# rchikhi/rust-seq2kminmers

Hardware: AMD Instinct MI355X
Metric: input bases/s (Gbp/s) for k-min-mer extraction, l=31 k=10 d=0.01 (higher is better)
Workload: dtype u32

## Files before the change

rust-seq2kminmers_amd/csrc/s2k_tile_impl.h:

```cpp
#pragma once
#include "s2k_dev.h"
#include "s2k_static_l.h"

#include <cstdlib>
#include <mutex>
#include <type_traits>

namespace s2k {
namespace {

#ifndef S2K_TW
#define S2K_TW 12
#endif
#ifndef S2K_TW_REG
#ifdef S2K_PROFILE
#define S2K_TW_REG 12
#else
#define S2K_TW_REG 16
#endif
#endif
template <bool HPC> constexpr int tw() { return HPC ? S2K_TW : S2K_TW_REG; }
template <bool HPC> constexpr int waves_per_simd() { return tw<HPC>() / 4; }
static_assert(S2K_TW % 4 == 0 && S2K_TW_REG % 4 == 0, "whole waves per SIMD");
constexpr int HS_OFF = 16;
constexpr int BUF_BYTES = HS_OFF + TILE_BASES + 128;
#ifndef S2K_CAPP
#define S2K_CAPP 16
#endif
constexpr int CAPP = S2K_CAPP;
constexpr int NPC = TILE_T / CAPP;
constexpr int MAX_L_TILED = 64;
#ifndef S2K_LISTCAP
#define S2K_LISTCAP 256
#endif
#ifndef S2K_JOBCAP
#define S2K_JOBCAP 32
#endif
#ifndef S2K_REDERIVE_GROUP
#define S2K_REDERIVE_GROUP 8
#endif
constexpr int LISTCAP_REG = S2K_TW_REG > 12 ? 216 : S2K_LISTCAP;
constexpr int LISTCAP_HPC = 192;
template <bool HPC> constexpr int listcap() { return HPC ? LISTCAP_HPC : LISTCAP_REG; }
template <bool HPC> constexpr int jobcap() { return !HPC && S2K_TW_REG > 12 ? 16 : S2K_JOBCAP; }
#ifndef S2K_REG_LA
#define S2K_REG_LA 1
#endif
#ifndef S2K_HPC_LA
#define S2K_HPC_LA 2
#endif
constexpr int REG_LA = S2K_REG_LA;
constexpr int HPC_LA = S2K_HPC_LA;
constexpr int NBL = 32;
template <bool DESC> constexpr int stores_per_round() { return DESC ? 1 : 3; }
static_assert(NBL == META_SEGS, "TileMeta keeps NBL segment starts");
constexpr int NPRE = 10;

#ifndef S2K_SD_SHIFT
#define S2K_SD_SHIFT 6
#endif
constexpr int ROW_W = 6, ROW_PFX = 4, ROW_CUM = 5, N_ROWS = 66, SD_SHIFT = S2K_SD_SHIFT;
struct HpcLds {
    uint32_t row[N_ROWS][ROW_W];
    uint32_t halo_pos[64];
    uint8_t sd[SD_SHIFT == 6 ? 160 : 288];
};
static_assert(sizeof(HpcLds) % 16 == 0, "the tile buffer behind it is read 16 bytes at a time");
struct NoHpcLds {};

template <bool HPC>
struct alignas(16) WaveLdsT : std::conditional<HPC, HpcLds, NoHpcLds>::type {
    uint8_t buf[BUF_BYTES];
    uint16_t list[listcap<HPC>()];
    uint16_t jobx[jobcap<HPC>()];
    uint16_t jobslot[jobcap<HPC>()];
    int16_t hb[NBL];
    uint16_t rs16[NBL];
};
#ifdef S2K_PROFILE
typedef __attribute__((address_space(3))) unsigned long long *ph_ptr_t;
constexpr int PROFILE_LDS_BYTES = 16 * 16 * 8;
#else
typedef uint64_t *ph_ptr_t;
constexpr int PROFILE_LDS_BYTES = 0;
#endif
constexpr int SEED_TABLE_BYTES = 2 * 256 * 8;
#ifndef S2K_SEL8
#define S2K_SEL8 1
#endif
constexpr int TABLE_BYTES = SEED_TABLE_BYTES;
constexpr int SEL8_OFF = SEED_TABLE_BYTES, SEL8_BYTES = S2K_SEL8 ? 256 * 8 : 0;
#ifndef S2K_PASS2_ACC
#define S2K_PASS2_ACC 1
#endif
static_assert(!S2K_PASS2_ACC || S2K_SEL8, "pass 2 reads its v_perm_b32 selectors from sel8");
#ifndef S2K_LPH
#define S2K_LPH 0
#endif
#ifndef S2K_WARM2
#define S2K_WARM2 1
#endif
constexpr int WARM_OFF = SEL8_OFF + SEL8_BYTES, WARM_BYTES = S2K_WARM2 ? 256 * 8 : 0;
template <bool HPC> constexpr int table_bytes() { return SEED_TABLE_BYTES + (HPC ? SEL8_BYTES + WARM_BYTES : 0); }
template <bool HPC>
constexpr int block_lds_bytes() { return table_bytes<HPC>() + tw<HPC>() * (int)sizeof(WaveLdsT<HPC>) + PROFILE_LDS_BYTES; }
#ifndef S2K_EXPERIMENT
static_assert(block_lds_bytes<true>() <= 160 * 1024 && block_lds_bytes<false>() <= 160 * 1024, "the block of a CU must fit its 160 KiB of LDS");
#endif

__device__ inline uint32_t wave_incl_scan(uint32_t v, int lane) {
    (void)lane;
    uint32_t t;
    t = (uint32_t)__builtin_amdgcn_update_dpp(0, (int)v, 0x111, 0xf, 0xf, false);
    uint32_t a = v + t;
    t = (uint32_t)__builtin_amdgcn_update_dpp(0, (int)v, 0x112, 0xf, 0xf, false);
    a += t;
    t = (uint32_t)__builtin_amdgcn_update_dpp(0, (int)v, 0x113, 0xf, 0xf, false);
    a += t;
// ... 6 lines not shown
    t = (uint32_t)__builtin_amdgcn_update_dpp(0, (int)a, 0x143, 0xc, 0xf, false);
    a += t;
    return a;
}
__device__ inline uint32_t wave_incl_max(uint32_t v) {
    uint32_t t, a;
    t = (uint32_t)__builtin_amdgcn_update_dpp(0, (int)v, 0x111, 0xf, 0xf, false);
    a = v > t ? v : t;
    t = (uint32_t)__builtin_amdgcn_update_dpp(0, (int)v, 0x112, 0xf, 0xf, false);
    a = a > t ? a : t;
    t = (uint32_t)__builtin_amdgcn_update_dpp(0, (int)v, 0x113, 0xf, 0xf, false);
    a = a > t ? a : t;
    t = (uint32_t)__builtin_amdgcn_update_dpp(0, (int)a, 0x114, 0xf, 0xe, false);
    a = a > t ? a : t;
    t = (uint32_t)__builtin_amdgcn_update_dpp(0, (int)a, 0x118, 0xf, 0xc, false);
    a = a > t ? a : t;
    t = (uint32_t)__builtin_amdgcn_update_dpp(0, (int)a, 0x142, 0xa, 0xf, false);
    a = a > t ? a : t;
    t = (uint32_t)__builtin_amdgcn_update_dpp(0, (int)a, 0x143, 0xc, 0xf, false);
    a = a > t ? a : t;
    return a;
}
__device__ inline uint32_t bcast(uint32_t v, int src) {
    return (uint32_t)__builtin_amdgcn_readlane((int)v, __builtin_amdgcn_readfirstlane(src));
}

__device__ inline uint32_t select_nth_32(uint32_t w, uint32_t n) {
    uint32_t r = 0, c;
    c = __popc(w & 0xFFFFu); if (n >= c) { n -= c; r += 16; w >>= 16; }
    c = __popc(w & 0xFFu);   if (n >= c) { n -= c; r += 8;  w >>= 8; }
    c = __popc(w & 0xFu);    if (n >= c) { n -= c; r += 4;  w >>= 4; }
    c = __popc(w & 0x3u);    if (n >= c) { n -= c; r += 2;  w >>= 2; }
    c = w & 1u;              if (n >= c) { r += 1; }
    return r;
}
__device__ __forceinline__ uint32_t select_nth_32_lut(uint32_t w, uint32_t n) {
    typedef __attribute__((address_space(3))) const uint8_t *lds_cu8;
    uint32_t r = 0, c;
    c = __popc(w & 0xFFFFu); if (n >= c) { n -= c; r += 16; w >>= 16; }
    c = __popc(w & 0xFFu);   if (n >= c) { n -= c; r += 8;  w >>= 8; }
    return r + reinterpret_cast<lds_cu8>((uint32_t)SEL8_OFF)[8u * (w & 0xFFu) + n];
}
__device__ __forceinline__ uint32_t mad24(uint32_t a, uint32_t b, uint32_t c) {
    uint32_t r;
    asm("v_mad_u32_u24 %0, %1, %2, %3" : "=v"(r) : "v"(a), "s"(b), "v"(c));
    return r;
}
__device__ __forceinline__ uint32_t div_tq(uint32_t x, uint32_t rcp) { return __umul24(x >> 4, rcp) >> 16; }
static_assert(TILE_T == 144, "div_tile_t's reciprocal is that of 144");
__device__ __forceinline__ uint32_t div_tile_t(uint32_t x) { return __umul24(x, 3641u) >> 19; }
__device__ __forceinline__ uint32_t bits_below(int v) {
    const int t = v < 0 ? 0 : (v > 32 ? 32 : v);
    return (uint32_t)(1ull << (uint32_t)t) - 1u;
}
__device__ __forceinline__ uint32_t heads_before_word(uint32_t cum, uint32_t g) {
    return __builtin_amdgcn_perm(cum, 0u, g + 0x0C0C0C03u);
}
__device__ __forceinline__ uint32_t word_of_head(uint32_t cum, uint32_t n) {
    uint32_t g = 0;
    asm("v_cmp_ge_u32_sdwa vcc, %1, %2 src0_sel:DWORD src1_sel:BYTE_0\n\t"
        "v_addc_co_u32_e32 %0, vcc, 0, %0, vcc\n\t"
        "v_cmp_ge_u32_sdwa vcc, %1, %2 src0_sel:DWORD src1_sel:BYTE_1\n\t"
        "v_addc_co_u32_e32 %0, vcc, 0, %0, vcc\n\t"
        "v_cmp_ge_u32_sdwa vcc, %1, %2 src0_sel:DWORD src1_sel:BYTE_2\n\t"
        "v_addc_co_u32_e32 %0, vcc, 0, %0, vcc\n\t"
        "v_cmp_ge_u32_sdwa vcc, %1, %2 src0_sel:DWORD src1_sel:BYTE_3\n\t"
        "v_addc_co_u32_e32 %0, vcc, 0, %0, vcc"
        : "+v"(g)
        : "v"(n), "v"(cum)
        : "vcc");
    return g;
}
template <int BYTE>
__device__ __forceinline__ uint32_t byte_x8(uint32_t w) {
    uint32_t off;
    if constexpr (BYTE == 0) asm("v_lshlrev_b32_sdwa %0, %1, %2 dst_sel:DWORD dst_unused:UNUSED_PAD src0_sel:DWORD src1_sel:BYTE_0" : "=v"(off) : "v"(3u), "v"(w));
    if constexpr (BYTE == 1) asm("v_lshlrev_b32_sdwa %0, %1, %2 dst_sel:DWORD dst_unused:UNUSED_PAD src0_sel:DWORD src1_sel:BYTE_1" : "=v"(off) : "v"(3u), "v"(w));
    if constexpr (BYTE == 2) asm("v_lshlrev_b32_sdwa %0, %1, %2 dst_sel:DWORD dst_unused:UNUSED_PAD src0_sel:DWORD src1_sel:BYTE_2" : "=v"(off) : "v"(3u), "v"(w));
    if constexpr (BYTE == 3) asm("v_lshlrev_b32_sdwa %0, %1, %2 dst_sel:DWORD dst_unused:UNUSED_PAD src0_sel:DWORD src1_sel:BYTE_3" : "=v"(off) : "v"(3u), "v"(w));
    return off;
}
template <int TABLE_OFF>
__device__ __forceinline__ uint2 seed_pair(uint32_t off) {
#ifdef HX_NOLDS
    return make_uint2(off, off);
#endif
    typedef __attribute__((address_space(3))) const unsigned long long lds_cu64;
    const unsigned long long v = *reinterpret_cast<lds_cu64 *>(off + TABLE_OFF);
    return make_uint2((uint32_t)v, (uint32_t)(v >> 32));
}
__device__ __forceinline__ uint2 tab_in(const uint2 *tab, uint32_t c) { return tab[c]; }
__device__ __forceinline__ uint2 tab_out(const uint2 *tab, uint32_t c) { return tab[256 + c]; }

__device__ __forceinline__ void hit_track(uint32_t hv, uint32_t bound, uint32_t &cap, uint32_t &bits) {
#ifdef HX_NOTRACK
    bits ^= hv;
    return;
#endif
    asm("v_cmp_ge_u32_e32 vcc, %2, %3\n\t"
        "v_cndmask_b32_e32 %0, %0, %3, vcc\n\t"
        "v_addc_co_u32_e32 %1, vcc, %1, %1, vcc"
        : "+v"(cap), "+v"(bits)
        : "s"(bound), "v"(hv)
        : "vcc");
}
template <int P>
// ... 513 lines not shown
__device__ __forceinline__ uint32_t heads_before_raw(const WL &S, uint32_t rel) {
    const uint32_t o = div_tile_t(rel), wi = rel - __umul24(o, (uint32_t)TILE_T), g = wi >> 5;
    const uint2 pc = *reinterpret_cast<const uint2 *>(&S.row[o][ROW_PFX]);
    const uint32_t wd = S.row[o][g];
    return (pc.x >> 16) + heads_before_word(pc.y, g) + __popc(wd & ((1u << (wi & 31u)) - 1u));
}

__device__ __forceinline__ uint32_t lookback_heads(const uint32_t *W, uint64_t t, int lane, Counts *counts, uint32_t early, bool &dead) {
    uint32_t sum = 0;
    if (dead) return 0;
    for (uint64_t tb = t;;) {
        const bool exists = tb >= 1 + (uint64_t)lane;
        const uint32_t *p = W + (exists ? tb - 1 - (uint64_t)lane : 0);
        uint32_t w = HW_VALID;
        int fs = 64;
        for (int polls = 0;; polls++) {
            if (exists) w = (polls == 0 && tb == t) ? early : __hip_atomic_load(p, __ATOMIC_RELAXED, __HIP_MEMORY_SCOPE_AGENT);
            const uint64_t valid = __ballot((w & HW_VALID) != 0u);
            const uint64_t stop = __ballot((w & HW_VALID) != 0u && (w & HW_PASS) == 0u);
            fs = stop ? __builtin_ctzll(stop) : 64;
            const uint64_t need = fs >= 63 ? ~0ull : ((2ull << fs) - 1ull);
            if ((valid & need) == need) break;
            const bool anybody = (polls & 63) == 63 && __hip_atomic_load(&counts->need_runs, __ATOMIC_RELAXED, __HIP_MEMORY_SCOPE_AGENT) != 0u;
            if (polls >= 4096 || __builtin_amdgcn_readfirstlane((int)anybody)) {
                if (lane == 0) counts->need_runs = 1;
                dead = true;
                return 0;
            }
            __builtin_amdgcn_s_sleep(16);
        }
        const uint32_t mine = (lane <= fs) ? (w & HW_COUNT) : 0u;
        sum += bcast(wave_incl_scan(mine, lane), 63);
        if (fs < 64) break;
        tb -= 64;
    }
    return sum;
}

template <class WL>
__device__ __forceinline__ void publish_tile_heads(uint32_t *W, uint64_t t, const WL &S, uint32_t nh, uint64_t t0, uint32_t tile_len,
                                                   bool any_start, uint64_t last_start, bool first_begins_here, int lane) {
    uint32_t word;
    if (!any_start) {
        word = HW_VALID | (first_begins_here ? 0u : HW_PASS) | nh;
    } else if (last_start >= t0 + tile_len) {
        word = HW_VALID;
    } else {
        const uint32_t c = heads_before_raw(S, (uint32_t)(last_start - t0));
        word = HW_VALID | (nh - c);
    }
    if (lane == 0) __hip_atomic_store(W + t, word, __ATOMIC_RELAXED, __HIP_MEMORY_SCOPE_AGENT);
}

template <int L, bool HPC, bool DESC, class WL, class IssueNext>
__device__ __forceinline__ uint32_t dense_phase(IssueNext &&issue_next, WL &S, const uint8_t *D, const uint2 *tab,
                                                const uint64_t *__restrict__ read_off, uint64_t n_reads, uint64_t t,
                                                uint64_t t0, uint32_t tile_len, uint32_t nh, uint32_t halo_n,
                                                uint32_t Tq, uint32_t rcpTq, uint32_t l, uint32_t r0, uint32_t r1, uint64_t bpos0,
                                                uint64_t rs0, int lane, const Records &rec, uint64_t *pool_cursor,
                                                uint32_t *mn_cnt, Counts *counts, uint64_t &base, const Sem &sem,
                                                unsigned long long *__restrict__ d_agg, TileMeta *__restrict__ d_meta, uint32_t K1,
                                                const uint32_t (&caps)[NPC], const uint32_t (&raw)[5], uint32_t lb_early,
                                                bool &lb_dead, ph_ptr_t ph, uint64_t &stamp) {
    constexpr int LISTCAP = listcap<HPC>();
    const uint32_t wclr = HPC ? (sem.keep_last ? l - 1 : l) : l - 1;
    const uint32_t tql = __umul24(Tq, (uint32_t)lane);
    uint32_t vm[5];
    {
        int vc = (int)nh - (int)tql;
#pragma unroll
        for (int d = 0; d < 5; d++) {
            vm[d] = raw[d] & bits_below(vc - 32 * d);
        }
    }
    const uint64_t tile_end = t0 + tile_len;
    uint32_t nb = 0;
    const bool many = (r1 - r0) > (uint32_t)(NBL - 2);
    bool ext_at_end = false;
    {
        uint64_t bpos = bpos0;
        uint64_t chunk_prev = rs0;
        int32_t hb_carry = 0;
        for (uint32_t c0 = 0;; c0 += 64) {
            const bool internal = bpos > t0 && bpos < tile_end;
            const bool external = bpos >= tile_end;
            const uint64_t em = __ballot(external);
            const int first_ext = em ? __builtin_ctzll(em) : 64;
            int32_t HB = 0x7FFFFFFF;
            if (internal || (external && lane == first_ext)) {
                if constexpr (HPC) {
                    if (bpos < tile_end) {
                        HB = (int32_t)heads_before_raw(S, (uint32_t)(bpos - t0));
                    } else {
                        HB = -1;
                    }
                } else {
                    const uint64_t rel = bpos - t0;
                    HB = rel > 0x3FFFFFFFull ? 0x3FFFFFFF : (int32_t)rel;
                }
            }
            if constexpr (HPC) {
                if (em) {
                    const uint64_t eb = ((uint64_t)bcast((uint32_t)(bpos >> 32), first_ext) << 32) | bcast((uint32_t)bpos, first_ext);
                    if (eb >= tile_end) {
                        const uint64_t relb = eb - t0;
                        const bool before = (uint32_t)lane < halo_n && (uint64_t)S.halo_pos[lane] < relb;
                        const int32_t hbx = (int32_t)(nh + (uint32_t)__popcll(__ballot(before)));
                        if (lane == first_ext) HB = hbx;
                    }
                }
            }
            uint64_t pstart = 0;
            uint32_t wextra = 0;
            if constexpr (HPC) {
                if (sem.tail_quirk) {
                    pstart = ((uint64_t)__shfl_up((uint32_t)(bpos >> 32), 1) << 32) | __shfl_up((uint32_t)bpos, 1);
                    if (lane == 0) pstart = chunk_prev;
                    const bool bnd = (internal || (external && lane == first_ext)) && bpos != ~0ull;
                    uint32_t Rr = 0;
                    if (sem.read_runs) {
                        if (bnd) Rr = sem.read_runs[(uint64_t)r0 + c0 + lane];
                    } else {
                        int32_t hprev = (int32_t)__shfl_up((uint32_t)HB, 1);
                        if (lane == 0) hprev = c0 == 0 ? 0 : hb_carry;
                        Rr = (uint32_t)(HB - hprev);
                        const bool began_before = c0 == 0 && !(t0 == 0 || rs0 == t0);
                        const bool reach = bnd && lane == 0 && began_before && HB - (int32_t)(wclr + 16u) < (int32_t)nh;
                        if (__ballot(reach)) {
                            const int32_t hb0 = (int32_t)bcast((uint32_t)HB, 0);
                            const int lo = hb0 - (int)wclr - 16 - (int)tql, hi = hb0 - (int)wclr - 1 - (int)tql;
                            uint32_t inwin = 0;
                            if (hi >= 0 && lo < (int)Tq) {
// ... 53 lines not shown
                    const uint32_t hx = bcast((uint32_t)(pstart - t0), z);
                    const int rel = (int)hx - (int)tql;
                    if (rel >= 0 && rel < (int)Tq) {
#pragma unroll
                        for (int d = 0; d < 5; d++)
                            if ((rel >> 5) == d) vm[d] &= ~(1u << (rel & 31));
                    }
                }
                chunk_prev = ((uint64_t)bcast((uint32_t)(bpos >> 32), 63) << 32) | bcast((uint32_t)bpos, 63);
            }
            if (!many && internal && c0 + lane < (uint32_t)(NBL - 1)) {
                S.hb[c0 + lane] = (int16_t)HB;
                S.rs16[c0 + lane + 1] = (uint16_t)(bpos - t0);
            }
            nb += (uint32_t)__popcll(__ballot(internal));
            if (em) {
                const uint64_t ebq = ((uint64_t)bcast((uint32_t)(bpos >> 32), first_ext) << 32) | bcast((uint32_t)bpos, first_ext);
                ext_at_end = ebq == tile_end;
                break;
            }
            const uint64_t ri = (uint64_t)r0 + 1 + c0 + 64 + lane;
            bpos = ri <= n_reads ? read_off[ri] : ~0ull;
            __builtin_amdgcn_s_waitcnt(0x0F70);
        }
    }
    S2K_STAMP(3);
    const uint32_t cnt = __popc(vm[0]) + __popc(vm[1]) + __popc(vm[2]) + __popc(vm[3]) + __popc(vm[4]);
    const uint32_t incl = wave_incl_scan(cnt, lane);
    const uint32_t myoff = incl - cnt;
    const uint32_t N = bcast(incl, 63);
    base = t * rec.slab_cap;
    bool dropped = false;
    if (N > rec.slab_cap) {
        uint64_t got = 0;
        if (lane == 0) got = atomicAdd(rec.ovf_cursor, (unsigned long long)N);
        got = ((uint64_t)bcast((uint32_t)(got >> 32), 0) << 32) | bcast((uint32_t)got, 0);
        base = rec.ovf_base + got;
        if (base + N > rec.capacity) {
            if (lane == 0) {
                counts->pool_overflow = 1;
                atomicMax((unsigned long long *)&counts->pool_needed, (unsigned long long)(got + N));
            }
            base = 0;
            dropped = true;
        }
    }
    if constexpr (!DESC) {
        if (N == 0 || dropped) {
            issue_next(0u, base);
            return 0;
        }
    }
    uint32_t mine = 0, segstart = 0;
    if (!many) {
        uint32_t below_prev = 0;
        for (uint32_t i = 0; i <= nb; i++) {
            uint32_t below = N;
            if (i < nb) {
                const int lim = S.hb[i] - (int)tql;
                uint32_t c = 0;
#pragma unroll
                for (int d = 0; d < 5; d++) {
                    c += __popc(vm[d] & bits_below(lim - 32 * d));
                }
                const int hbi = S.hb[i];
                const int lb = hbi <= 0 ? 0 : ((uint32_t)hbi >= Tq * 64u ? 63 : (int)div_tq((uint32_t)hbi, rcpTq));
                below = bcast(myoff + c, lb);
            }
            if ((uint32_t)lane == i) {
                mine = below - below_prev;
                segstart = below_prev;
            }
            below_prev = below;
        }
        if constexpr (!DESC)
            if ((uint32_t)lane <= nb && mine) atomicAdd(&mn_cnt[r0 + lane], mine);
    }
    if constexpr (DESC) {
        if (many) {
            if (lane == 0) counts->need_legacy = 1;
            issue_next(0u, base);
            return 0;
        }
        const bool dep = !(t0 == 0 || rs0 == t0);
        const uint32_t m_first = bcast(mine, 0), m_last = bcast(mine, (int)nb);
        uint32_t wfix = (uint32_t)lane <= nb && mine > K1 ? mine - K1 : 0u;
        if (lane == 0 && dep) wfix = 0;
        uint32_t Cfix;
        if (nb <= 2u) Cfix = bcast(wfix, 0) + (nb >= 1u ? bcast(wfix, 1) : 0u) + (nb >= 2u ? bcast(wfix, 2) : 0u);
        else Cfix = bcast(wave_incl_scan(wfix, lane), 63);
        const bool pass = dep && nb == 0 && !ext_at_end;
        const uint32_t q_out = ext_at_end ? 0u : (m_last < K1 ? m_last : K1);
        if (lane == 0) {
            d_agg[t] = agg_pack(m_first, Cfix, dropped ? 0u : N, q_out, dep, pass);
            TileMeta *m = &d_meta[t];
            m->rec_base = base;
            m->rs0 = rs0;
            m->r0 = r0;
            m->nb = (uint16_t)nb;
            m->nrd = (uint16_t)(r1 - r0);
        }
        if ((uint32_t)lane <= nb) {
            d_meta[t].segstart[lane] = (uint16_t)segstart;
            if (lane) d_meta[t].rs16[lane] = S.rs16[lane];
        }
        if (N == 0 || dropped || (sem.dbg_skip & 128)) {
            issue_next(0u, base);
            return 0;
        }
    }
    uint32_t njobs = 0;
    auto flush_jobs = [&]() {
        wave_sync();
        const uint32_t part = (uint32_t)lane & 3u;
        const uint32_t per = (l + 3u) >> 2;
        const uint32_t i0 = per * part;
        for (uint32_t j0 = 0; j0 < njobs; j0 += 16) {
            const uint32_t job = j0 + ((uint32_t)lane >> 2);
            const bool act = job < njobs;
            const uint8_t *q = D + (act ? S.jobx[job] : 0) + i0;
            uint32_t f = 0, r = 0;
            if constexpr (L > 0) {
                constexpr uint32_t PER = (L + 3) / 4;
                constexpr uint32_t GRP = S2K_REDERIVE_GROUP;
#pragma unroll
                for (uint32_t h0 = 0; h0 < PER; h0 += GRP) {
                    uint32_t by[GRP];
                    uint2 ti[GRP];
#pragma unroll
                    for (uint32_t ii = 0; ii < GRP; ii++)
                        if (h0 + ii < PER) by[ii] = q[h0 + ii];
#pragma unroll
                    for (uint32_t ii = 0; ii < GRP; ii++)
                        if (h0 + ii < PER) ti[ii] = tab_in(tab, by[ii]);
                    uint32_t tf[GRP], tr[GRP];
#pragma unroll
                    for (uint32_t ii = 0; ii < GRP; ii++) {
                        tf[ii] = tr[ii] = 0u;
                        if (h0 + ii < PER) {
                            const uint32_t i = i0 + h0 + ii, rot = (uint32_t)L - 1u - i;
                            const bool valid = 3 * PER + h0 + ii < (uint32_t)L || i < (uint32_t)L;
                            tf[ii] = valid ? rotl32(ti[ii].x, rot) : 0u;
                            tr[ii] = valid ? rotr32(ti[ii].y, rot) : 0u;
                        }
                    }
#pragma unroll
                    for (uint32_t ii = 0; ii < GRP; ii += 4) {
                        f = xor3(xor3(f, tf[ii], tf[ii + 1]), tf[ii + 2], tf[ii + 3]);
                        r = xor3(xor3(r, tr[ii], tr[ii + 1]), tr[ii + 2], tr[ii + 3]);
                    }
                    if (GRP < PER) __builtin_amdgcn_sched_barrier(0);
                }
            } else {
                for (uint32_t ii = 0; ii < per; ii++) {
                    const uint32_t i = i0 + ii;
                    if (i < l) {
                        const uint2 ti = tab_in(tab, q[ii]);
                        f ^= rotl32(ti.x, l - 1 - i);
// ... 304 lines not shown
    ph_ptr_t ph = reinterpret_cast<ph_ptr_t>((uint32_t)(table_bytes<HPC>() + TW * sizeof(WL) + (size_t)w * 128));
    if (lane0 < 16) ph[lane0] = 0;
    wave_sync();
#else
    ph_ptr_t ph = nullptr;
#endif

    auto is_full = [&](uint64_t tt) { return (tt + 1) * (uint64_t)TILE_BASES + 128 <= n_bases; };
    uint32_t prevb = 0;
    bool have_pre = false;
    typedef __attribute__((address_space(3))) uint8_t lds_u8s;
    auto prefetch = [&](uint64_t tt) {
        static_assert(NPRE == 10, "4 + 4 + 1 wave-wide loads of 1 KiB and one of 128 B");
        const uint8_t *g = bases + tt * (uint64_t)TILE_BASES + 16 * lane;
        const uint32_t lbase = (uint32_t)(uintptr_t)(lds_u8s *)D;
        uint32_t save;
#pragma unroll
        for (int grp = 0; grp < 2; grp++) {
            const uint8_t *pg = g + 4096 * grp;
            const uint32_t m = (uint32_t)__builtin_amdgcn_readfirstlane((int)(lbase + 4096u * grp));
            asm volatile("s_mov_b32 %0, m0\n\ts_mov_b32 m0, %2\n\ts_nop 0\n\t"
                         "global_load_lds_dwordx4 %1, off\n\tglobal_load_lds_dwordx4 %1, off offset:1024\n\t"
                         "global_load_lds_dwordx4 %1, off offset:2048\n\tglobal_load_lds_dwordx4 %1, off offset:3072\n\t"
                         "s_mov_b32 m0, %0"
                         : "=&s"(save) : "v"(pg), "s"(m) : "memory");
        }
        const uint8_t *pg = g + 8192;
        const uint32_t m = (uint32_t)__builtin_amdgcn_readfirstlane((int)(lbase + 8192u));
        asm volatile("s_mov_b32 %0, m0\n\ts_mov_b32 m0, %2\n\ts_nop 0\n\tglobal_load_lds_dwordx4 %1, off\n\ts_mov_b32 m0, %0"
                     : "=&s"(save) : "v"(pg), "s"(m) : "memory");
        if (lane < 8)
            asm volatile("s_mov_b32 %0, m0\n\ts_mov_b32 m0, %2\n\ts_nop 0\n\tglobal_load_lds_dwordx4 %1, off offset:1024\n\ts_mov_b32 m0, %0"
                         : "=&s"(save) : "v"(pg), "s"(m) : "memory");
    };
    auto byte_before = [&](uint64_t tt) -> uint32_t { return tt > 0 ? (uint32_t)bases[tt * (uint64_t)TILE_BASES - 1] : 0u; };
    auto read_entries = [&](uint32_t rr0, uint64_t &bp, uint64_t &rs) {
        const uint64_t bri = (uint64_t)rr0 + 1 + lane;
        bp = bri <= n_reads ? read_off[bri] : ~0ull;
        rs = read_off[rr0];
    };
    uint32_t r0 = cold_args().tile_read0[t], r1 = cold_args().tile_read0[t + 1];
    uint64_t bpos0, rs0;
    read_entries(r0, bpos0, rs0);
    if (is_full(t)) prevb = byte_before(t);
    __builtin_amdgcn_s_waitcnt(0x0F70);
    if (is_full(t)) {
        prefetch(t);
        have_pre = true;
    }
    uint32_t stores_after_dma = 0;
    uint64_t tn = t + n_waves, tnn = t + 2 * n_waves;
    const uint64_t dyn0 = tile_begin + 3 * n_waves;
    const uint32_t cur_g = (uint32_t)((blockIdx.x * TW + w + blockIdx.x / (TILE_CURSORS / 4)) % TILE_CURSORS);
    auto cursors = [&]() { return (unsigned int *)(cold_args().pool_cursor + 16); };
    uint32_t r0n = 0, r1n = 0;
    if (tn < n_tiles) {
        r0n = cold_args().tile_read0[tn];
        r1n = cold_args().tile_read0[tn + 1];
    }

    uint32_t prio_iter = 0;
    bool lb_dead = sem.tile_heads != nullptr && __builtin_amdgcn_readfirstlane((int)cold_args().counts->need_runs) != 0;
    for (; t < n_tiles;) {
        lane = lane0;
        asm volatile("" : "+v"(lane));
        asm volatile("" : "+s"(cold_p));
        asm volatile("" : "+s"(bases));
        asm volatile("" : "+s"(wl_off));
        WL &S = *reinterpret_cast<WL *>(smem + wl_off);
        D = S.buf + HS_OFF;
        if (sem.tile_heads) {
            switch ((prio_iter++ + (uint32_t)(w >> 2)) % 3u) {
                case 0: __builtin_amdgcn_s_setprio(0); break;
                case 1: __builtin_amdgcn_s_setprio(1); break;
                default: __builtin_amdgcn_s_setprio(2); break;
            }
        }
        const uint64_t t0 = t * (uint64_t)TILE_BASES;
        const uint64_t rem = n_bases - t0;
        const uint32_t avail = rem > (uint64_t)(TILE_BASES + 128) ? (uint32_t)(TILE_BASES + 128) : (uint32_t)rem;
        const uint32_t tile_len = rem > (uint64_t)TILE_BASES ? (uint32_t)TILE_BASES : (uint32_t)rem;
        uint32_t l16_tile = 16 * lane;
        if (__builtin_amdgcn_readfirstlane((int)have_pre)) {
            constexpr int SPR = stores_per_round<DESC>();
            asm volatile("; S2K_MARK counted_wait per_round=%0" ::"i"(SPR));
            switch (__builtin_amdgcn_readfirstlane((int)stores_after_dma)) {
                case 1 * SPR: __builtin_amdgcn_s_waitcnt(0x0F70 | (1 * SPR)); break;
                case 2 * SPR: __builtin_amdgcn_s_waitcnt(0x0F70 | (2 * SPR)); break;
                case 3 * SPR: __builtin_amdgcn_s_waitcnt(0x0F70 | (3 * SPR)); break;
                case 4 * SPR: __builtin_amdgcn_s_waitcnt(0x0F70 | (4 * SPR)); break;
                default: __builtin_amdgcn_s_waitcnt(0x0F70); break;
            }
            asm volatile("" ::: "memory");
            __builtin_amdgcn_wave_barrier();
        } else {
            const uint8_t *g = bases + t0;
            uint32_t l16o = l16_tile;
            asm volatile("" : "+v"(l16o));
            for (int r = 0; r < NPRE; r++) {
                const uint32_t off = l16o + 1024 * r;
                if (r == NPRE - 1 && lane >= 8) break;
                uint4 v = make_uint4(0, 0, 0, 0);
                if (off + 16 <= avail) {
                    v = *reinterpret_cast<const uint4 *>(g + off);
                } else if (off < avail) {
                    uint32_t tmp[4] = {0, 0, 0, 0};
                    for (uint32_t b = 0; off + b < avail && b < 16; b++) tmp[b >> 2] |= (uint32_t)g[off + b] << (8 * (b & 3));
                    v = make_uint4(tmp[0], tmp[1], tmp[2], tmp[3]);
                }
                *reinterpret_cast<uint4 *>(D + off) = v;
            }
            prevb = t0 > 0 ? (uint32_t)bases[t0 - 1] : 0u;
            __builtin_amdgcn_s_waitcnt(0x0F70);
        }
        const uint32_t cr0 = r0, cr1 = r1, cprev = prevb;
        uint32_t took = 0;
        if (lane == 0 && tnn < n_tiles) took = atomicAdd(&cursors()[32 * cur_g], 1u);
        uint64_t bposn = ~0ull, rs0n = 0;
        uint32_t r0nn = 0, r1nn = 0, prevbn = 0;
        const uint64_t brin = (uint64_t)r0n + 1 + lane;
// ... 62 lines not shown
        };
        const uint32_t Tq = 16 * np;
        uint32_t N = 0;
        uint64_t base = 0;
        uint32_t caps[NPC], raw[5];
#pragma unroll
        for (int g2 = 0; g2 < NPC; g2++) caps[g2] = 0;
#pragma unroll
        for (int g2 = 0; g2 < 5; g2++) raw[g2] = 0;
        if (nh != 0 && sem.enabled) {
#ifndef EXP_NOHASH
            if (!(sem.dbg_skip & 1)) hash_stage<L, HPC>(D, tab, sem.bound_le, lane, l, np, caps, raw);
#endif
            wave_sync();
            __builtin_amdgcn_sched_barrier(0);
#ifdef S2K_XCAL
            {
                uint32_t dv = (uint32_t)lane, dv2 = (uint32_t)lane + 3u, ds = (uint32_t)t;
                (void)dv; (void)dv2; (void)ds;
#pragma unroll
                for (int i_ = 0; i_ < 64; i_++) {
#if S2K_XCAL == 1
                    asm volatile("v_xor_b32 %0, %0, %1\n\tv_xor_b32 %1, %1, %0\n\tv_xor_b32 %0, %0, %1\n\tv_xor_b32 %1, %1, %0" : "+v"(dv), "+v"(dv2));
#elif S2K_XCAL == 2
                    asm volatile("v_alignbit_b32 %0, %0, %1, 7\n\tv_alignbit_b32 %1, %1, %0, 9\n\tv_alignbit_b32 %0, %0, %1, 7\n\tv_alignbit_b32 %1, %1, %0, 9" : "+v"(dv), "+v"(dv2));
#elif S2K_XCAL == 3
                    asm volatile("s_add_u32 %0, %0, 1\n\ts_xor_b32 %0, %0, 5\n\ts_add_u32 %0, %0, 3\n\ts_xor_b32 %0, %0, 9" : "+s"(ds));
#elif S2K_XCAL == 4
                    asm volatile("ds_read_b32 %0, %2\n\tds_read_b32 %1, %2 offset:4\n\tds_read_b32 %0, %2 offset:8\n\tds_read_b32 %1, %2 offset:12" : "=v"(dv), "=v"(dv2) : "v"(4u * (uint32_t)lane) : "memory");
#elif S2K_XCAL == 6
                    if (i_ < 16) asm volatile("ds_read_b32 %0, %2\n\tds_read_b32 %1, %2 offset:4\n\tds_read_b32 %0, %2 offset:8\n\tds_read_b32 %1, %2 offset:12" : "=v"(dv), "=v"(dv2) : "v"(4u * ((uint32_t)lane & 7u) + 128u * ((uint32_t)lane >> 3)) : "memory");
#elif S2K_XCAL == 7
                    if (i_ < 16) asm volatile("ds_read_b32 %0, %2\n\tds_read_b32 %1, %2 offset:4\n\tds_read_b32 %0, %2 offset:8\n\tds_read_b32 %1, %2 offset:12" : "=v"(dv), "=v"(dv2) : "v"(4u * (uint32_t)lane) : "memory");
#elif S2K_XCAL == 8
                    if (i_ < 16) asm volatile("ds_read_b32 %0, %2\n\tds_read_b32 %1, %2 offset:4\n\tds_read_b32 %0, %2 offset:8\n\tds_read_b32 %1, %2 offset:12" : "=v"(dv), "=v"(dv2) : "v"(4u * ((uint32_t)lane & 1u) + 128u * ((uint32_t)lane >> 1)) : "memory");
#elif S2K_XCAL == 5
                    asm volatile("v_min_u32 %0, %0, %1\n\tv_max_u32 %1, %1, %0\n\tv_min_u32 %0, %0, %1\n\tv_max_u32 %1, %1, %0" : "+v"(dv), "+v"(dv2));
#endif
                }
                asm volatile("s_waitcnt lgkmcnt(0)" ::: "memory");
                asm volatile("" ::"v"(dv), "v"(dv2), "s"(ds));
            }
#endif
            S2K_STAMP(2);
        }
        __builtin_amdgcn_s_waitcnt(0x0F70);
        if (brin > n_reads) bposn = ~0ull;
        rs0n = ((uint64_t)(uint32_t)__builtin_amdgcn_readfirstlane((int)(uint32_t)(rs0n >> 32)) << 32) |
               (uint32_t)__builtin_amdgcn_readfirstlane((int)(uint32_t)rs0n);
        r0nn = (uint32_t)__builtin_amdgcn_readfirstlane((int)r0nn);
        r1nn = (uint32_t)__builtin_amdgcn_readfirstlane((int)r1nn);
        prevbn = (uint32_t)__builtin_amdgcn_readfirstlane((int)prevbn);
        uint64_t drawn = ~0ull;
        if (tnn < n_tiles)
            drawn = dyn0 + cur_g + (uint64_t)TILE_CURSORS * (uint32_t)__builtin_amdgcn_readfirstlane((int)took);
        bool issued = false;
        auto issue_once = [&](uint32_t n_rec, uint64_t rec_base) {
            if (!issued) issue_next(n_rec, rec_base);
            issued = true;
        };
        int lane_d = lane;
        asm volatile("" : "+v"(lane_d));
        if (DESC || (nh != 0 && sem.enabled)) {
#ifndef EXP_NODENSE
            if (!(sem.dbg_skip & 2))
                N = dense_phase<L, HPC, DESC>(issue_once, S, D, tab, read_off, n_reads, t, t0, tile_len, nh, halo_n, Tq, rcpTq, l, cr0, cr1,
                                           bpos0, rs0, lane_d, cold_args().rec, cold_args().pool_cursor, cold_args().mn_cnt,
                                           cold_args().counts, base, sem, cold_args().d_agg, cold_args().d_meta, cold_args().K1,
                                           caps, raw, lb_early, lb_dead, ph, stamp);
#endif
            S2K_STAMP(5);
        }
        issue_once(0, 0);
        {
            const bool many = (cr1 - cr0) > (uint32_t)(NBL - 2) || (sem.dbg_skip & 16) != 0;
            constexpr uint32_t LISTCAP = (uint32_t)listcap<HPC>();
            const uint32_t last = N == 0 ? 0u : N - ((N - 1) / LISTCAP) * LISTCAP;
            stores_after_dma = many ? 0u : (uint32_t)stores_per_round<DESC>() * ((last + 63u) / 64u);
        }
        wave_sync();
        r0 = r0n; r1 = r1n; bpos0 = bposn; rs0 = rs0n; r0n = r0nn; r1n = r1nn; prevb = prevbn;
        t = tn;
        tn = tnn;
        if (tnn < n_tiles) tnn = drawn;
        S2K_STAMP(6);
    }
#ifdef S2K_PROFILE
    if ((sem.dbg_skip & 8) && lane == 0)
        for (int i = 0; i < 16; i++) atomicAdd((unsigned long long *)&cold_args().counts->dbg_cycles[blockIdx.x & 63][i], (unsigned long long)ph[i]);
#endif
#ifdef S2K_DEBUG_KNOBS
    if ((sem.dbg_skip & 32) && lane == 0) {
        const unsigned long long now = __builtin_amdgcn_s_memrealtime();
        atomicMax((unsigned long long *)&cold_args().counts->dbg_cycles[0][0], now);
        atomicMax((unsigned long long *)&cold_args().counts->dbg_cycles[0][1], ~now);
        atomicAdd((unsigned long long *)&cold_args().counts->dbg_cycles[1][0], (unsigned long long)(__builtin_amdgcn_s_memtime() - dbg_mt0));
        atomicAdd((unsigned long long *)&cold_args().counts->dbg_cycles[1][1], (unsigned long long)(now - dbg_rt0));
        const uint32_t wid = blockIdx.x * TW + w;
        if (wid < 4096) {
            cold_args().counts->dbg_wave[wid][0] = now;
            cold_args().counts->dbg_wave[wid][1] = ((uint64_t)__builtin_amdgcn_s_getreg((20 | (0 << 6) | (31 << 11))) << 32) | (uint32_t)__builtin_amdgcn_s_getreg((4 | (0 << 6) | (31 << 11)));
        }
    }
#endif
}

#ifndef S2K_STREAM_BUILD
#define S2K_STREAM_BUILD 0
#endif
#if S2K_STREAM_BUILD
#ifndef S2K_STREAM_DEFAULT
#define S2K_STREAM_DEFAULT 0
#endif
#ifndef S2K_STREAM_TW
#define S2K_STREAM_TW 16
#endif
#ifndef S2K_STREAM_BPC
#define S2K_STREAM_BPC 1
#endif
// ... 43 lines not shown
        const uint64_t bri = (uint64_t)r0 + 1 + lane;
        bpos0 = bri <= n_reads ? read_off[bri] : ~0ull;
        rs0 = read_off[r0];
    }
    uint64_t tn = t + n_waves, tnn = t + 2 * n_waves;
    const uint64_t dyn0 = tile_begin + 3 * n_waves;
    const uint32_t cur_g = (uint32_t)((blockIdx.x * TW + w + blockIdx.x / (TILE_CURSORS / 4)) % TILE_CURSORS);
    unsigned int *const cursors = (unsigned int *)(pool_cursor + 16);
    uint32_t r0n = 0, r1n = 0;
    if (tn < n_tiles) {
        r0n = tile_read0[tn];
        r1n = tile_read0[tn + 1];
    }
    bool lb_dead = false;
    for (; t < n_tiles;) {
        lane = lane0;
        asm volatile("" : "+v"(lane));
        const uint64_t t0 = t * (uint64_t)TILE_BASES;
        const uint32_t cr0 = r0, cr1 = r1;
        uint32_t took = 0;
        if (lane == 0 && tnn < n_tiles) took = atomicAdd(&cursors[32 * cur_g], 1u);
        uint64_t bposn = ~0ull, rs0n = 0;
        uint32_t r0nn = 0, r1nn = 0;
        const uint64_t brin = (uint64_t)r0n + 1 + lane;
        uint32_t vzero = 0;
        asm volatile("" : "+v"(vzero));
        if (tn < n_tiles) {
            bposn = read_off[brin <= n_reads ? brin : n_reads];
            rs0n = read_off[(uint64_t)r0n + vzero];
            if (tnn < n_tiles) {
                r0nn = tile_read0[tnn + vzero];
                r1nn = tile_read0[tnn + 1 + vzero];
            }
        }
        uint32_t caps[NPC], raw[5];
#pragma unroll
        for (int g2 = 0; g2 < NPC; g2++) caps[g2] = 0;
#pragma unroll
        for (int g2 = 0; g2 < 5; g2++) raw[g2] = 0;
        const uint8_t *D = bases + t0;
        if (sem.enabled) hash_loop_static<L, REG_LA, false, true>(D, sem.bound_le, lane, TILE_T / 16, caps, raw);
        __builtin_amdgcn_sched_barrier(0);
        __builtin_amdgcn_s_waitcnt(0x0F70);
        if (brin > n_reads) bposn = ~0ull;
        rs0n = ((uint64_t)(uint32_t)__builtin_amdgcn_readfirstlane((int)(uint32_t)(rs0n >> 32)) << 32) | (uint32_t)__builtin_amdgcn_readfirstlane((int)(uint32_t)rs0n);
        r0nn = (uint32_t)__builtin_amdgcn_readfirstlane((int)r0nn);
        r1nn = (uint32_t)__builtin_amdgcn_readfirstlane((int)r1nn);
        uint64_t drawn = ~0ull;
        if (tnn < n_tiles) drawn = dyn0 + cur_g + (uint64_t)TILE_CURSORS * (uint32_t)__builtin_amdgcn_readfirstlane((int)took);
        int lane_d = lane;
        asm volatile("" : "+v"(lane_d));
        uint64_t base = 0;
        auto no_issue = [](uint32_t, uint64_t) {};
        (void)dense_phase<L, false, true>(no_issue, S, D, tab, read_off, n_reads, t, t0, (uint32_t)TILE_BASES, (uint32_t)TILE_BASES, 0u, (uint32_t)TILE_T, 7282u, l,
                                          cr0, cr1, bpos0, rs0, lane_d, rec, pool_cursor, (uint32_t *)nullptr, counts, base, sem, d_agg, d_meta, K1, caps, raw, 0u,
                                          lb_dead, ph, stamp);
        wave_sync();
        r0 = r0n; r1 = r1n; bpos0 = bposn; rs0 = rs0n; r0n = r0nn; r1n = r1nn;
        t = tn;
        tn = tnn;
        if (tnn < n_tiles) tnn = drawn;
    }
}

template <int L>
hipError_t launch_stream_l(hipStream_t st, const uint8_t *bases, const uint64_t *read_off, uint64_t n_reads, uint64_t n_bases, uint64_t n_tiles_full,
                           const uint32_t *tile_read0, Sem sem, Records rec, uint64_t *pool_cursor, Counts *counts, const Desc *desc, uint64_t tile_begin) {
    if constexpr (L > 0) {
        auto kern = stream_minimizer_kernel<L>;
        constexpr int lds = stream_lds_bytes();
        constexpr int MAX_DEV = 64;
        static int n_cu_d[MAX_DEV] = {0};
        static std::mutex cache_mu;
        int dev = 0;
        S2K_HIP_CHECK(hipGetDevice(&dev));
        if (dev < 0 || dev >= MAX_DEV) return hipErrorInvalidDevice;
        std::lock_guard<std::mutex> lk(cache_mu);
        if (n_cu_d[dev] == 0) {
            S2K_HIP_CHECK(hipFuncSetAttribute(reinterpret_cast<const void *>(kern), hipFuncAttributeMaxDynamicSharedMemorySize, lds));
            hipDeviceProp_t prop;
            S2K_HIP_CHECK(hipGetDeviceProperties(&prop, dev));
            n_cu_d[dev] = prop.multiProcessorCount;
        }
        uint64_t blocks = (n_tiles_full - tile_begin + STREAM_TW - 1) / STREAM_TW;
        const uint64_t resident = (uint64_t)n_cu_d[dev] * STREAM_BPC;
        if (blocks > resident) blocks = resident;
        hipLaunchKernelGGL(kern, dim3((unsigned)blocks), dim3(64 * STREAM_TW), lds, st, bases, read_off, n_reads, n_bases, n_tiles_full, tile_read0, sem, rec,
                           pool_cursor, counts, desc->agg, desc->meta, desc->k - 1u, tile_begin);
        return hipGetLastError();
    } else {
        return hipErrorInvalidValue;
    }
}
#endif

template <int L, bool HPC, bool DESC, int MODE>
hipError_t launch_tiles_lh(hipStream_t st, const uint8_t *bases, const uint64_t *read_off, uint64_t n_reads, uint64_t n_bases,
                           uint64_t n_tiles, const uint32_t *tile_read0, Sem sem, Records rec, uint64_t *pool_cursor,
                           uint64_t *tile_rec_off, uint32_t *tile_cnt, uint32_t *mn_cnt, Counts *counts, const Desc *desc, uint64_t tile_begin) {
    auto kern = tile_minimizer_kernel<L, HPC, DESC, MODE>;
    constexpr int TW = tw<HPC>();
    const int lds = block_lds_bytes<HPC>();
    constexpr int MAX_DEV = 64;
    static int n_cu_d[MAX_DEV] = {0}, per_cu_d[MAX_DEV] = {0};
    static std::mutex cache_mu;
    int dev = 0;
    S2K_HIP_CHECK(hipGetDevice(&dev));
// ... 75 lines not shown
```

Baseline: 1844.

## Add fast path in dense phase for tiles with at most one read boundary

Adds a specialised path in dense_phase for the common case where a tile holds at most one internal read boundary. It computes the boundary masks and head counts directly from two broadcast boundary offsets instead of running the general 64-lane boundary loop with LDS hb/rs16 arrays, and writes the per-tile metadata compactly. It also moves the dynamic cursor base into LDS for the HPC variant to reduce register pressure. The cost is a second code path, with bit-packed state that must stay consistent with the general path.

```diff
diff --git a/rust-seq2kminmers_amd/csrc/s2k_tile_impl.h b/rust-seq2kminmers_amd/csrc/s2k_tile_impl.h
--- a/rust-seq2kminmers_amd/csrc/s2k_tile_impl.h
+++ b/rust-seq2kminmers_amd/csrc/s2k_tile_impl.h
@@ -64,6 +64,7 @@
     uint32_t row[N_ROWS][ROW_W];
     uint32_t halo_pos[64];
     uint8_t sd[SD_SHIFT == 6 ? 160 : 288];
+    unsigned long long dyn_g, pad_;
 };
 static_assert(sizeof(HpcLds) % 16 == 0, "the tile buffer behind it is read 16 bytes at a time");
 struct NoHpcLds {};
@@ -176,6 +177,19 @@
 __device__ __forceinline__ uint32_t bits_below(int v) {
     const int t = v < 0 ? 0 : (v > 32 ? 32 : v);
     return (uint32_t)(1ull << (uint32_t)t) - 1u;
+}
+template <bool NARROW>
+__device__ __forceinline__ void clear_range(uint32_t (&vm)[5], int lo, int hi, uint32_t tql) {
+    const int a = lo - (int)tql, b = hi - (int)tql;
+#pragma unroll
+    for (int d = 0; d < 5; d++) {
+        if constexpr (NARROW) {
+            const int ca = min(max(a, 32 * d), 32 * d + 32), cb = min(max(b, 32 * d), 32 * d + 32);
+            vm[d] &= ~((((uint32_t)1 << (uint32_t)(cb - ca)) - 1u) << ((uint32_t)ca & 31u));
+        } else {
+            vm[d] &= ~(bits_below(b - 32 * d) & ~bits_below(a - 32 * d));
+        }
+    }
 }
 __device__ __forceinline__ uint32_t heads_before_word(uint32_t cum, uint32_t g) {
     return __builtin_amdgcn_perm(cum, 0u, g + 0x0C0C0C03u);
@@ -795,7 +809,7 @@
     if (lane == 0) __hip_atomic_store(W + t, word, __ATOMIC_RELAXED, __HIP_MEMORY_SCOPE_AGENT);
 }
 
-template <int L, bool HPC, bool DESC, class WL, class IssueNext>
+template <int L, bool HPC, bool DESC, int MODE, class WL, class IssueNext>
 __device__ __forceinline__ uint32_t dense_phase(IssueNext &&issue_next, WL &S, const uint8_t *D, const uint2 *tab,
                                                 const uint64_t *__restrict__ read_off, uint64_t n_reads, uint64_t t,
                                                 uint64_t t0, uint32_t tile_len, uint32_t nh, uint32_t halo_n,
@@ -820,7 +834,51 @@
     uint32_t nb = 0;
     const bool many = (r1 - r0) > (uint32_t)(NBL - 2);
     bool ext_at_end = false;
-    {
+    constexpr bool FEW_OK = DESC && MODE != TILE_MODE_RUNTIME;
+    constexpr uint32_t FEW_BIT = 0x80000000u;
+    static_assert(TILE_BASES < (1 << 14), "the few path packs a raw offset and an HB of the tile into 14 bits each");
+    uint32_t fr0 = 0, fr1 = 0;
+    if constexpr (FEW_OK) {
+        uint64_t bp = bpos0;
+        asm volatile("" : "+v"(bp));
+        const uint32_t brel = bp <= t0 ? 0u : (bp - t0 > 0xFFFFFFFFull ? 0xFFFFFFFFu : (uint32_t)(bp - t0));
+        fr0 = bcast(brel, 0);
+        fr1 = bcast(brel, 1);
+    }
+    if (FEW_OK && !many && fr0 != 0u && fr1 >= tile_len) {
+        int32_t hb_in = 0;
+        const uint32_t fnb = fr0 < tile_len ? 1u : 0u;
+        const uint32_t eb = fnb ? fr1 : fr0;
+        const bool fext = eb == tile_len;
+        constexpr bool NARROW = L > 0 && L < 32;
+        if (fnb) {
+            if constexpr (HPC) hb_in = __builtin_amdgcn_readfirstlane((int)heads_before_raw(S, fr0));
+            else hb_in = (int32_t)fr0;
+            clear_range<NARROW>(vm, hb_in - (int)wclr, hb_in, tql);
+        }
+        int32_t hb_ex;
+        if constexpr (HPC) {
+            const bool before = (uint32_t)lane < halo_n && S.halo_pos[lane] < eb;
+            hb_ex = (int32_t)(nh + (uint32_t)__popcll(__ballot(before)));
+        } else {
+            hb_ex = eb > 0x3FFFFFFFu ? 0x3FFFFFFF : (int32_t)eb;
+        }
+        if (hb_ex - (int)wclr < (int)nh) clear_range<NARROW>(vm, hb_ex - (int)wclr, hb_ex, tql);
+        if constexpr (!HPC) {
+#pragma unroll
+            for (int e = 0; e < 2; e++) {
+                const bool exact = e == 0 ? rs0 == t0 && fr0 == l : fr0 < tile_len && fr1 != 0xFFFFFFFFu && fr1 - fr0 == l;
+                const int rel = (int)(e == 0 ? 0u : fr0) - (int)tql;
+                if (exact && rel >= 0 && rel < (int)Tq) {
+#pragma unroll
+                    for (int d = 0; d < 5; d++)
+                        if ((rel >> 5) == d) vm[d] &= ~(1u << (rel & 31));
+                }
+            }
+        }
+        nb = FEW_BIT | (fext ? 1u << 29 : 0u) | (fnb ? fr0 << 15 | (uint32_t)hb_in << 1 | 1u : 0u);
+        asm volatile("" : "+s"(nb));
+    } else {
         uint64_t bpos = bpos0;
         uint64_t chunk_prev = rs0;
         int32_t hb_carry = 0;
@@ -980,58 +1038,94 @@
         }
     }
     uint32_t mine = 0, segstart = 0;
-    if (!many) {
-        uint32_t below_prev = 0;
-        for (uint32_t i = 0; i <= nb; i++) {
+    if (nb & FEW_BIT) {
+        if constexpr (FEW_OK) {
+            const uint32_t fst = nb;
+            nb = fst & 1u;
+            const bool ext_at_end = (fst >> 29) & 1u;
             uint32_t below = N;
-            if (i < nb) {
-                const int lim = S.hb[i] - (int)tql;
+            if (nb) {
+                const int hb_in = (int)((fst >> 1) & 0x3FFFu);
+                const int lb = hb_in <= 0 ? 0 : ((uint32_t)hb_in >= Tq * 64u ? 63 : (int)div_tq((uint32_t)hb_in, rcpTq));
+                const int lim = hb_in - (int)(Tq * (uint32_t)lb);
                 uint32_t c = 0;
 #pragma unroll
-                for (int d = 0; d < 5; d++) {
-                    c += __popc(vm[d] & bits_below(lim - 32 * d));
-                }
-                const int hbi = S.hb[i];
-                const int lb = hbi <= 0 ? 0 : ((uint32_t)hbi >= Tq * 64u ? 63 : (int)div_tq((uint32_t)hbi, rcpTq));
+                for (int d = 0; d < 5; d++) c += __popc(vm[d] & bits_below(lim - 32 * d));
                 below = bcast(myoff + c, lb);
             }
-            if ((uint32_t)lane == i) {
-                mine = below - below_prev;
-                segstart = below_prev;
-            }
-            below_prev = below;
-        }
-        if constexpr (!DESC)
-            if ((uint32_t)lane <= nb && mine) atomicAdd(&mn_cnt[r0 + lane], mine);
+            const bool dep = !(t0 == 0 || rs0 == t0);
+            const uint32_t m_first = below, m_last = N - (nb ? below : 0u);
+            const uint32_t Cfix = (!dep && m_first > K1 ? m_first - K1 : 0u) + (nb && m_last > K1 ? m_last - K1 : 0u);
+            const bool pass = dep && nb == 0 && !ext_at_end;
+            const uint32_t q_out = ext_at_end ? 0u : (m_last < K1 ? m_last : K1);
+            if (lane == 0) {
+                d_agg[t] = agg_pack(m_first, Cfix, dropped ? 0u : N, q_out, dep, pass);
+                TileMeta *m = &d_meta[t];
+                m->rec_base = base;
+                m->rs0 = rs0;
+                m->r0 = r0;
+                m->nb = (uint16_t)nb;
+                m->nrd = (uint16_t)(r1 - r0);
+                *reinterpret_cast<uint32_t *>(&m->segstart[0]) = nb ? below << 16 : 0u;
+                if (nb) m->rs16[1] = (uint16_t)((fst >> 15) & 0x3FFFu);
+            }
+        }
+    } else {
+        if (!many) {
+            uint32_t below_prev = 0;
+            for (uint32_t i = 0; i <= nb; i++) {
+                uint32_t below = N;
+                if (i < nb) {
+                    const int lim = S.hb[i] - (int)tql;
+                    uint32_t c = 0;
+#pragma unroll
+                    for (int d = 0; d < 5; d++) {
+                        c += __popc(vm[d] & bits_below(lim - 32 * d));
+                    }
+                    const int hbi = S.hb[i];
+                    const int lb = hbi <= 0 ? 0 : ((uint32_t)hbi >= Tq * 64u ? 63 : (int)div_tq((uint32_t)hbi, rcpTq));
+                    below = bcast(myoff + c, lb);
+                }
+                if ((uint32_t)lane == i) {
+                    mine = below - below_prev;
+                    segstart = below_prev;
+                }
+                below_prev = below;
+            }
+            if constexpr (!DESC)
+                if ((uint32_t)lane <= nb && mine) atomicAdd(&mn_cnt[r0 + lane], mine);
+        }
+        if constexpr (DESC) {
+            if (many) {
+                if (lane == 0) counts->need_legacy = 1;
+                issue_next(0u, base);
+                return 0;
+            }
+            const bool dep = !(t0 == 0 || rs0 == t0);
+            const uint32_t m_first = bcast(mine, 0), m_last = bcast(mine, (int)nb);
+            uint32_t wfix = (uint32_t)lane <= nb && mine > K1 ? mine - K1 : 0u;
+            if (lane == 0 && dep) wfix = 0;
+            uint32_t Cfix;
+            if (nb <= 2u) Cfix = bcast(wfix, 0) + (nb >= 1u ? bcast(wfix, 1) : 0u) + (nb >= 2u ? bcast(wfix, 2) : 0u);
+            else Cfix = bcast(wave_incl_scan(wfix, lane), 63);
+            const bool pass = dep && nb == 0 && !ext_at_end;
+            const uint32_t q_out = ext_at_end ? 0u : (m_last < K1 ? m_last : K1);
+            if (lane == 0) {
+                d_agg[t] = agg_pack(m_first, Cfix, dropped ? 0u : N, q_out, dep, pass);
+                TileMeta *m = &d_meta[t];
+                m->rec_base = base;
+                m->rs0 = rs0;
+                m->r0 = r0;
+                m->nb = (uint16_t)nb;
+                m->nrd = (uint16_t)(r1 - r0);
+            }
+            if ((uint32_t)lane <= nb) {
+                d_meta[t].segstart[lane] = (uint16_t)segstart;
+                if (lane) d_meta[t].rs16[lane] = S.rs16[lane];
+            }
+        }
     }
     if constexpr (DESC) {
-        if (many) {
-            if (lane == 0) counts->need_legacy = 1;
-            issue_next(0u, base);
-            return 0;
-        }
-        const bool dep = !(t0 == 0 || rs0 == t0);
-        const uint32_t m_first = bcast(mine, 0), m_last = bcast(mine, (int)nb);
-        uint32_t wfix = (uint32_t)lane <= nb && mine > K1 ? mine - K1 : 0u;
-        if (lane == 0 && dep) wfix = 0;
-        uint32_t Cfix;
-        if (nb <= 2u) Cfix = bcast(wfix, 0) + (nb >= 1u ? bcast(wfix, 1) : 0u) + (nb >= 2u ? bcast(wfix, 2) : 0u);
-        else Cfix = bcast(wave_incl_scan(wfix, lane), 63);
-        const bool pass = dep && nb == 0 && !ext_at_end;
-        const uint32_t q_out = ext_at_end ? 0u : (m_last < K1 ? m_last : K1);
-        if (lane == 0) {
-            d_agg[t] = agg_pack(m_first, Cfix, dropped ? 0u : N, q_out, dep, pass);
-            TileMeta *m = &d_meta[t];
-            m->rec_base = base;
-            m->rs0 = rs0;
-            m->r0 = r0;
-            m->nb = (uint16_t)nb;
-            m->nrd = (uint16_t)(r1 - r0);
-        }
-        if ((uint32_t)lane <= nb) {
-            d_meta[t].segstart[lane] = (uint16_t)segstart;
-            if (lane) d_meta[t].rs16[lane] = S.rs16[lane];
-        }
         if (N == 0 || dropped || (sem.dbg_skip & 128)) {
             issue_next(0u, base);
             return 0;
@@ -1442,6 +1536,8 @@
     uint64_t tn = t + n_waves, tnn = t + 2 * n_waves;
     const uint64_t dyn0 = tile_begin + 3 * n_waves;
     const uint32_t cur_g = (uint32_t)((blockIdx.x * TW + w + blockIdx.x / (TILE_CURSORS / 4)) % TILE_CURSORS);
+    if constexpr (HPC)
+        if (lane0 == 0) reinterpret_cast<WL *>(smem + wl_off)->dyn_g = dyn0 + cur_g;
     auto cursors = [&]() { return (unsigned int *)(cold_args().pool_cursor + 16); };
     uint32_t r0n = 0, r1n = 0;
     if (tn < n_tiles) {
@@ -1456,6 +1552,7 @@
         asm volatile("" : "+v"(lane));
         asm volatile("" : "+s"(cold_p));
         asm volatile("" : "+s"(bases));
+        asm volatile("" : "+s"(read_off));
         asm volatile("" : "+s"(wl_off));
         WL &S = *reinterpret_cast<WL *>(smem + wl_off);
         D = S.buf + HS_OFF;
@@ -1624,8 +1721,11 @@
         r1nn = (uint32_t)__builtin_amdgcn_readfirstlane((int)r1nn);
         prevbn = (uint32_t)__builtin_amdgcn_readfirstlane((int)prevbn);
         uint64_t drawn = ~0ull;
-        if (tnn < n_tiles)
-            drawn = dyn0 + cur_g + (uint64_t)TILE_CURSORS * (uint32_t)__builtin_amdgcn_readfirstlane((int)took);
+        if (tnn < n_tiles) {
+            uint64_t dg = dyn0 + cur_g;
+            if constexpr (HPC) dg = S.dyn_g;
+            drawn = dg + (uint64_t)TILE_CURSORS * (uint32_t)__builtin_amdgcn_readfirstlane((int)took);
+        }
         bool issued = false;
         auto issue_once = [&](uint32_t n_rec, uint64_t rec_base) {
             if (!issued) issue_next(n_rec, rec_base);
@@ -1636,7 +1736,7 @@
         if (DESC || (nh != 0 && sem.enabled)) {
 #ifndef EXP_NODENSE
             if (!(sem.dbg_skip & 2))
-                N = dense_phase<L, HPC, DESC>(issue_once, S, D, tab, read_off, n_reads, t, t0, tile_len, nh, halo_n, Tq, rcpTq, l, cr0, cr1,
+                N = dense_phase<L, HPC, DESC, MODE>(issue_once, S, D, tab, read_off, n_reads, t, t0, tile_len, nh, halo_n, Tq, rcpTq, l, cr0, cr1,
                                            bpos0, rs0, lane_d, cold_args().rec, cold_args().pool_cursor, cold_args().mn_cnt,
                                            cold_args().counts, base, sem, cold_args().d_agg, cold_args().d_meta, cold_args().K1,
                                            caps, raw, lb_early, lb_dead, ph, stamp);
@@ -1786,7 +1886,7 @@
         asm volatile("" : "+v"(lane_d));
         uint64_t base = 0;
         auto no_issue = [](uint32_t, uint64_t) {};
-        (void)dense_phase<L, false, true>(no_issue, S, D, tab, read_off, n_reads, t, t0, (uint32_t)TILE_BASES, (uint32_t)TILE_BASES, 0u, (uint32_t)TILE_T, 7282u, l,
+        (void)dense_phase<L, false, true, TILE_MODE_RUNTIME>(no_issue, S, D, tab, read_off, n_reads, t, t0, (uint32_t)TILE_BASES, (uint32_t)TILE_BASES, 0u, (uint32_t)TILE_T, 7282u, l,
                                           cr0, cr1, bpos0, rs0, lane_d, rec, pool_cursor, (uint32_t *)nullptr, counts, base, sem, d_agg, d_meta, K1, caps, raw, 0u,
                                           lb_dead, ph, stamp);
         wave_sync();
```

Result: faster. 1864, median of 6 (+1.1%).
